# telin0411/multimodal_sequencing

Measured on AMD Instinct MI355X. Metric: multimodal steps/sec (fwd+bwd) at N=5 steps, seq=512, ViT-B/16; 1/2/4/8 GPU, higher is better.
Workload: dtype bf16; 1 GPU; config3: ViT-B/16 + 12x768 joint encoder + BERSON, N=5 steps, 20 pairs/story, pair seq 120+393=513; global_batch=32, stories_per_gpu=32, micro_batch=32, seq_len=513, parallelism=dp1

## Files before the change

multimodal_sequencing_amd/csrc/gemm256.hip:

```cpp
#include "gemm_common.h"

using namespace mmseq_gemm_detail;

namespace {

typedef unsigned short us;
__device__ __forceinline__ void ld8(const us* p, float* v) {
  const u16x8 u = *reinterpret_cast<const u16x8*>(p);
#pragma unroll
  for (int r = 0; r < 8; ++r) v[r] = bf2f(u[r]);
}
__device__ __forceinline__ void st8(us* p, const float* v) {
  u16x8 u;
#pragma unroll
  for (int r = 0; r < 8; ++r) u[r] = f2bf(v[r]);
  *reinterpret_cast<u16x8*>(p) = u;
}

struct EpiIn { u16x8 x; };
template <bool BWD, bool Q8 = false, bool CHK = true>
__device__ __forceinline__ EpiIn epi8_load(const GemmArgs& a, int m, int n) {
  EpiIn in;
  in.x = (u16x8){0, 0, 0, 0, 0, 0, 0, 0};
  if (CHK && (m >= a.M || n >= a.N)) return in;
  const int64_t off = (int64_t)m * (Q8 ? a.ldcb : a.ldc) + n;
  if (BWD) in.x = *reinterpret_cast<const u16x8*>(reinterpret_cast<const us*>(a.dact) + off);
  else if (a.resid) in.x = *reinterpret_cast<const u16x8*>(reinterpret_cast<const us*>(a.resid) + (int64_t)m * a.ldr + n);
  else if (a.accumulate) in.x = *reinterpret_cast<const u16x8*>(reinterpret_cast<const us*>(a.C) + off);
  return in;
}

struct EpiBias { f32x4 b0, b1; };
__device__ __forceinline__ EpiBias epi_bias(const GemmArgs& a, int n) {
  EpiBias b;
  b.b0 = b.b1 = (f32x4){0.f, 0.f, 0.f, 0.f};
  if (!a.bias || n >= a.N) return b;
  if ((((uintptr_t)a.bias) & 15) == 0) {
    b.b0 = *reinterpret_cast<const f32x4*>(a.bias + n);
    b.b1 = *reinterpret_cast<const f32x4*>(a.bias + n + 4);
  } else {
#pragma unroll
    for (int r = 0; r < 4; ++r) { b.b0[r] = a.bias[n + r]; b.b1[r] = a.bias[n + 4 + r]; }
  }
  asm volatile("" ::"v"(b.b0), "v"(b.b1));
  return b;
}

constexpr int DT_LO = 117 << 7;
constexpr int DT_N = 13 * 128;
__device__ __forceinline__ int dtab_index(unsigned short u) {
  const int a = min(max((int)(u & 0x7FFFu) - DT_LO, 0), DT_N - 1);
  return a + (int)(u >> 15) * DT_N;
}
template <int ACT>
__device__ __forceinline__ void dtab_fill(float MMSEQ_LDS* tab) {
  for (int e = threadIdx.x; e < 2 * DT_N; e += blockDim.x) {
    const unsigned short u = (unsigned short)(((e / DT_N) << 15) | (e % DT_N + DT_LO));
    tab[e] = act_bwd(ACT, bf2f(u));
  }
}

template <int ACT, bool BWD, bool XIN, bool DTAB = false, bool CHK = true>
__device__ __forceinline__ void epi8(const GemmArgs& a, int m, int n, f32x4 lo, f32x4 hi, const EpiIn& in,
                                     const EpiBias& bias, const float MMSEQ_LDS* dtab = nullptr) {
  if (CHK && (m >= a.M || n >= a.N)) return;
  float v[8];
  if (XIN) {
#pragma unroll
    for (int r = 0; r < 4; ++r) {
      v[r] = fmaf(lo[r], a.alpha, bias.b0[r]);
      v[4 + r] = fmaf(hi[r], a.alpha, bias.b1[r]);
    }
  } else {
    bias_alpha8(v, lo, hi, a.alpha, bias.b0, bias.b1);
  }
#ifdef MMSEQ_EPI_SINK
  const int64_t off = (int64_t)(m & 255) * a.ldc + n;
#else
  const int64_t off = (int64_t)m * a.ldc + n;
#endif
  if (BWD) {
    if (DTAB) {
#pragma unroll
      for (int r = 0; r < 8; ++r) v[r] *= dtab[dtab_index(in.x[r])];
    } else if (ACT == MMSEQ_ACT_GELU_ERF) {
#pragma unroll
      for (int r = 0; r < 8; ++r) v[r] *= gelu_sig_grad(bf2f(in.x[r]));
    } else {
#pragma unroll
      for (int r = 0; r < 8; ++r) v[r] *= act_bwd_fast(ACT, bf2f(in.x[r]));
    }
  } else if (ACT) {
    if (a.aux) st8(reinterpret_cast<us*>(a.aux) + off, v);
    if (ACT == MMSEQ_ACT_GELU_ERF) {
      gelu_sig8(v);
    } else {
#pragma unroll
      for (int r = 0; r < 8; ++r) v[r] = act_fwd_fast(ACT, v[r]);
    }
  }
  if (!BWD && a.drop.thr) {
    float dm[8];
    drop_mul_pairs<4>(a.drop, (uint64_t)m * a.N + n, dm);
#pragma unroll
    for (int r = 0; r < 8; ++r) v[r] *= dm[r];
  }
  if (XIN && !BWD) {
#pragma unroll
    for (int r = 0; r < 8; ++r) v[r] += bf2f(in.x[r]);
  }
  st8(reinterpret_cast<us*>(a.C) + off, v);
}

__device__ __forceinline__ void q8_scale_words(const GemmArgs& a, int mrow, int ncol,
                                               const uint8_t MMSEQ_LDS* sq, int lane) {
  const uint32_t w = *(const uint32_t MMSEQ_LDS*)(sq + 4 * lane);
  const int Mp = (a.M + 63) & ~63;
  if (mrow < Mp && ncol < a.N) {
    const int KB = a.N >> 5;
    const rsrc_t rq = make_rsrc(a.q8_scales, (int64_t)(Mp >> 6) * KB * 64);
    const uint32_t off = (uint32_t)(((mrow >> 6) * KB + (ncol >> 5)) * 64 + (mrow & 15) * 4);
    __builtin_amdgcn_raw_buffer_store_b32(w, rq, off, 0, 0);
  }
}
template <int ACT, bool BWD = false>
__device__ __forceinline__ void epi8_q8(const GemmArgs& a, int m, int n, int g, f32x4 lo, f32x4 hi,
                                        const EpiBias& bias, uint8_t MMSEQ_LDS* sqb,
                                        const EpiIn* din = nullptr,
                                        const float MMSEQ_LDS* dtab = nullptr) {
  float v[8];
  bias_alpha8(v, lo, hi, a.alpha, bias.b0, bias.b1);
  const bool in = m < a.M && n < a.N;
  const int64_t offb = (int64_t)m * a.ldcb + n;
  if (BWD) {
#pragma unroll
    for (int r = 0; r < 8; ++r) v[r] *= dtab[dtab_index(din->x[r])];
  } else {
    if (ACT && a.aux && in) st8(reinterpret_cast<us*>(a.aux) + offb, v);
    if (ACT == MMSEQ_ACT_GELU_ERF) {
      gelu_sig8(v);
    } else if (ACT) {
#pragma unroll
      for (int r = 0; r < 8; ++r) v[r] = act_fwd_fast(ACT, v[r]);
    }
  }
  float amax = 0.f;
#pragma unroll
  for (int r = 0; r < 8; ++r) {
    v[r] = bf2f(f2bf(v[r]));
    amax = fmaxf(amax, fabsf(v[r]));
  }
  if (a.cbf && in) st8(reinterpret_cast<us*>(a.cbf) + offb, v);
  {
    uint32_t u = __float_as_uint(amax);
    const auto r16 = __builtin_amdgcn_permlane16_swap(u, u, false, false);
    u = max(r16[0], r16[1]);
    const auto r32 = __builtin_amdgcn_permlane32_swap(u, u, false, false);
    amax = __uint_as_float(max(r32[0], r32[1]));
  }
  int e = amax > 0.f ? (int)((__float_as_uint(amax) >> 23) & 0xff) - 127 : -127;
  e = max(-127, min(127, e - 8));
  const float inv = ldexpf(1.f, -e);
  *sqb = (uint8_t)(m < a.M ? e + 127 : 0);
  if (!in) return;
  uint32_t w[2];
#pragma unroll
  for (int j = 0; j < 2; ++j) {
    const float s0 = fminf(448.f, fmaxf(-448.f, v[4 * j] * inv));
    const float s1 = fminf(448.f, fmaxf(-448.f, v[4 * j + 1] * inv));
    const float s2 = fminf(448.f, fmaxf(-448.f, v[4 * j + 2] * inv));
    const float s3 = fminf(448.f, fmaxf(-448.f, v[4 * j + 3] * inv));
    int pk = __builtin_amdgcn_cvt_pk_fp8_f32(s0, s1, 0, false);
    pk = __builtin_amdgcn_cvt_pk_fp8_f32(s2, s3, pk, true);
    w[j] = (uint32_t)pk;
  }
  typedef __attribute__((ext_vector_type(2))) unsigned int u32x2;
  *reinterpret_cast<u32x2*>(reinterpret_cast<uint8_t*>(a.C) + (int64_t)m * a.ldc + n) =
      (u32x2){w[0], w[1]};
}

constexpr int G_LDA_HALF = 16384;

#ifndef MMSEQ_NT_GROUP_M
#define MMSEQ_NT_GROUP_M 8
#endif
#ifndef MMSEQ_NT_GROUP_M_AUX
#define MMSEQ_NT_GROUP_M_AUX 16
#endif
__device__ __forceinline__ void tile_mn(int tile, int tiles_n, int ntiles, int& tm, int& tn,
                                        bool aux2 = false) {
  const int GM = tiles_n >= 8 ? (aux2 && tiles_n >= 12 ? MMSEQ_NT_GROUP_M_AUX : MMSEQ_NT_GROUP_M) : 1;
  if (GM <= 1) {
    tm = tile / tiles_n;
    tn = tile - tm * tiles_n;
    return;
  }
  const int tiles_m = ntiles / tiles_n;
  const int per = GM * tiles_n;
  const int grp = tile / per, first = grp * GM;
  const int gm = min(tiles_m - first, GM);
  const int r = tile - grp * per;
  tm = first + r % gm;
  tn = r / gm;
}

__device__ __forceinline__ int g8_of(int X, int q) {
  if (X == 0) return (q & 7) + ((q >> 3) << 4);
  if (X == 3) return 8 + (q & 7) + ((q >> 3) << 4);
  if (X == 1) return (q & 3) + ((q >> 2) << 3);
  return 4 + (q & 3) + ((q >> 2) << 3);
}

typedef __attribute__((ext_vector_type(8))) int i32x8;
typedef __attribute__((ext_vector_type(4))) int i32x4;
__device__ __forceinline__ i32x8 cat8(const bf16x8_t& lo, const bf16x8_t& hi) {
  const i32x4 l = __builtin_bit_cast(i32x4, lo), h = __builtin_bit_cast(i32x4, hi);
  return (i32x8){l[0], l[1], l[2], l[3], h[0], h[1], h[2], h[3]};
}

__device__ __forceinline__ void mfma_f8_acc(f32x4& c, const i32x8& a, const i32x8& b, uint32_t sa,
                                            uint32_t sb) {
  asm volatile("v_mfma_scale_f32_16x16x128_f8f6f4 %0, %1, %2, %0, %3, %4 op_sel_hi:[0,0,0]"
               : "+v"(c) : "v"(a), "v"(b), "v"(sa), "v"(sb));
}

template <int ACT, bool BWD, bool XIN, bool Q8 = false, bool F8 = false>
__global__ __launch_bounds__(512, 1) void gemm256_nt_kernel(GemmArgs a, int tiles_n, int ntiles,
                                                            int delay) {
  __shared__ __attribute__((aligned(16))) unsigned short
      smem[2 * 2 * G_LDA_HALF + (BWD ? 4 * DT_N : 0) + (F8 ? 2048 : 0) + 1024 + (Q8 ? 1024 : 0)];
  unsigned short* const sscale = smem + 2 * 2 * G_LDA_HALF + (BWD ? 4 * DT_N : 0);
  unsigned short* const sbias = smem + 2 * 2 * G_LDA_HALF + (BWD ? 4 * DT_N : 0) + (F8 ? 2048 : 0);
  const int tid = threadIdx.x, lane = tid & 63;
  const int wave = __builtin_amdgcn_readfirstlane(tid >> 6);
  uint8_t MMSEQ_LDS* const sq8 = (uint8_t MMSEQ_LDS*)(sbias + 1024) + wave * 256;
  const int wr = wave >> 2, wc = wave & 3;
  const int G = gridDim.x;
  const bool aux2 = ACT > 0 && !BWD && a.aux != nullptr;
  float MMSEQ_LDS* dtab = (float MMSEQ_LDS*)(smem + 2 * 2 * G_LDA_HALF);
  if (BWD) dtab_fill<ACT>(dtab);
  const int bid = blockIdx.x;
  const int first = xcd_item(bid, G);
  if (delay > 0 && first < ntiles && (ntiles - 1 - first) / G < (ntiles - 1) / G) {
    const uint64_t t0 = __builtin_amdgcn_s_memtime();
    while (__builtin_amdgcn_s_memtime() - t0 < (uint64_t)delay) __builtin_amdgcn_s_sleep(8);
  }
  const int nk = F8 ? a.K >> 7 : a.K >> 6;
  const int64_t lda_b = F8 ? a.lda : 2 * a.lda, ldb_b = F8 ? a.ldb : 2 * a.ldb;
  const int64_t kbytes = F8 ? a.K : 2 * a.K;
  const uint8_t* Ab = reinterpret_cast<const uint8_t*>(a.A);
  const uint8_t* Bb = reinterpret_cast<const uint8_t*>(a.B);
  const int KB32 = a.K >> 5;
  constexpr int LBUF = F8 ? G_LDA_HALF : 2 * G_LDA_HALF;
  constexpr int LOPB = F8 ? 2 * G_LDA_HALF : G_LDA_HALF;

  const int lr = lane >> 3, lc = lane & 7;
  const uint32_t offA0 = (uint32_t)(lr * lda_b + ((lc ^ (lane >> 4)) << 4));
  const uint32_t offA1 = (uint32_t)(lr * lda_b + ((lc ^ ((lane >> 4) | 4)) << 4));
  const uint32_t offB0 = (uint32_t)(lr * ldb_b + ((lc ^ ((lane >> 4) & 1)) << 4));
  const uint32_t offB1 = (uint32_t)(lr * ldb_b + ((lc ^ (((lane >> 4) & 1) | 2)) << 4));
  const uint32_t offB2 = (uint32_t)(lr * ldb_b + ((lc ^ (((lane >> 4) & 1) | 4)) << 4));
  const uint32_t offB3 = (uint32_t)(lr * ldb_b + ((lc ^ (((lane >> 4) & 1) | 6)) << 4));

  const rsrc_t rBias = make_rsrc(a.bias, a.bias ? (int64_t)a.N * 4 : 0);
  const rsrc_t rSA = make_rsrc(a.f8_sa, F8 ? a.f8_sa_bytes : 0);
  const rsrc_t rSB = make_rsrc(a.f8_sb, F8 ? a.f8_sb_bytes : 0);
  struct Sc { int ga, gb; };
  auto descs = [&](int tile, rsrc_t& ra, rsrc_t& rb, Sc& sc) {
    if (tile < ntiles) {
      int tm, tn;
      tile_mn(tile, tiles_n, ntiles, tm, tn, aux2);
      const int m0 = tm * 256, n0 = tn * 256;
      ra = make_rsrc(Ab + (int64_t)m0 * lda_b, (int64_t)(a.M - m0 - 1) * lda_b + kbytes);
      rb = make_rsrc(Bb + (int64_t)n0 * ldb_b, (int64_t)(a.N - n0 - 1) * ldb_b + kbytes);
      sc.ga = m0 >> 6;
      sc.gb = n0 >> 6;
    } else {
      ra = rb = make_rsrc(Ab, 0);
      sc.ga = (int)(a.f8_sa_bytes / 64 / (KB32 > 0 ? KB32 : 1));
      sc.gb = (int)(a.f8_sb_bytes / 64 / (KB32 > 0 ? KB32 : 1));
    }
  };
  rsrc_t rAc, rBc, rAn, rBn;
  Sc scc{}, scn{};
  descs(first, rAc, rBc, scc);
  descs(first + G, rAn, rBn, scn);

  auto stage = [&](int it, int kk, int X) {
    (void)it;
    const bool nxt = kk >= nk;
    if (nxt) kk -= nk;
    const bool isA = (X == 0 || X == 3);
    const rsrc_t r = isA ? (nxt ? rAn : rAc) : (nxt ? rBn : rBc);
    const int64_t ld = isA ? lda_b : ldb_b;
    unsigned short* img = smem + (kk & 1) * LBUF + (isA ? 0 : LOPB);
#pragma unroll
    for (int i = 0; i < 2; ++i) {
      const int q = wave * 2 + i;
      const int g8 = g8_of(X, q);
      const int gb = g8 & 3;
      const uint32_t lo = isA ? ((g8 & 1) ? offA1 : offA0)
                              : (gb == 0 ? offB0 : gb == 1 ? offB1 : gb == 2 ? offB2 : offB3);
      const uint32_t voff = lo + (uint32_t)(g8 * 8 * ld + kk * 128);
      dma16(r, img + g8 * 512, voff);
    }
    if (F8 && X == 3) {
      const bool sa = wave < 4;
      const int grp = (sa ? (nxt ? scn.ga : scc.ga) : (nxt ? scn.gb : scc.gb)) + (wave & 3);
      const uint32_t so = (uint32_t)(((int64_t)grp * KB32 + 4 * kk) * 64 + lane * 16);
      unsigned short* dst = sscale + (kk & 1) * 1024 + wave * 128;
      if (sa) {
        if (lane < 16) dma16(rSA, dst, so);
      } else {
        if (lane < 16) dma16(rSB, dst, so);
      }
    }
  };

  const int l15 = lane & 15;
  const int sw0 = ((lane >> 4) ^ (l15 >> 1)) << 3;
  const int sw1 = ((4 + (lane >> 4)) ^ (l15 >> 1)) << 3;
  const int arow = (wr * 128 + l15) * 64;
  const int hb = ((l15 >> 1) & 1) | ((l15 >> 2) << 1);
  const int swb0 = ((lane >> 4) ^ hb) << 3;
  const int swb1 = ((4 + (lane >> 4)) ^ hb) << 3;
  const int brow = LOPB + ((wc >> 1) * 128 + (wc & 1) * 64 + 8 * (l15 >> 2) + (l15 & 3)) * 64;
#define FR(base, t, ks) __builtin_bit_cast(bf16x8_t, *reinterpret_cast<const u16x8*>( \
      smem + (base) + (t) * 1024 + ((ks) ? sw1 : sw0)))
#define FRB(base, j, ks) __builtin_bit_cast(bf16x8_t, *reinterpret_cast<const u16x8*>( \
      smem + (base) + (4 * ((j) & 1) + 32 * ((j) >> 1)) * 64 + ((ks) ? swb1 : swb0)))

  uint32_t scA[2] = {0u, 0u}, scB[2] = {0u, 0u};
  const int scb_sh = 8 * (l15 >> 3);
  const uint8_t* scbase = reinterpret_cast<const uint8_t*>(sscale) + (lane >> 4) * 64;
  auto read_scales = [&](int h) {
    const uint8_t* sp = scbase + h * 2048;
    scA[0] = *reinterpret_cast<const uint32_t*>(sp + (wr * 2) * 256 + l15 * 4);
    scA[1] = *reinterpret_cast<const uint32_t*>(sp + (wr * 2 + 1) * 256 + l15 * 4);
    const int rb = 8 * ((l15 >> 2) & 1) + (l15 & 3);
    scB[0] = *reinterpret_cast<const uint32_t*>(sp + 1024 + wc * 256 + rb * 4);
    scB[1] = *reinterpret_cast<const uint32_t*>(sp + 1024 + wc * 256 + (rb + 4) * 4);
  };
#define QUAD(I0, I1, J0, J1)                                                                      \
  if (F8) {                                                                                       \
    uint32_t sa_[I1 - I0], sb_[J1 - J0];                                                          \
    _Pragma("unroll") for (int i = I0; i < I1; ++i) sa_[i - I0] = scA[i >> 2] >> (8 * (i & 3));   \
    _Pragma("unroll") for (int j = J0; j < J1; ++j)                                               \
      sb_[j - J0] = scB[j & 1] >> (scb_sh + 16 * (j >> 1));                                       \
        \
                                       \
    asm volatile("s_nop 4" ::"v"(sa_[0]), "v"(sa_[I1 - I0 - 1]), "v"(sb_[0]), "v"(sb_[J1 - J0 - 1])); \
    _Pragma("unroll") for (int i = I0; i < I1; ++i)                                               \
    _Pragma("unroll") for (int j = J0; j < J1; ++j)                                               \
      mfma_f8_acc(acc[i][j], fb8[j], fa8[i], sb_[j - J0], sa_[i - I0]);                           \
  } else {                                                                                        \
    _Pragma("unroll") for (int ks = 0; ks < 2; ++ks)                                              \
    _Pragma("unroll") for (int i = I0; i < I1; ++i)                                               \
    _Pragma("unroll") for (int j = J0; j < J1; ++j)                                               \
      acc[i][j] = __builtin_amdgcn_mfma_f32_16x16x32_bf16(fb[j][ks], fa[i][ks], acc[i][j], 0, 0, 0); \
  }

  int it = 0;
  if (first >= ntiles) return;
  stage(0, 0, 0); stage(0, 0, 1); stage(0, 0, 2); stage(0, 0, 3);
  stage(0, 1, 0); stage(0, 1, 1);
  asm volatile("s_waitcnt vmcnt(4)" ::: "memory");
  __builtin_amdgcn_s_barrier();
  if (wr) __builtin_amdgcn_s_barrier();

  f32x4 acc[8][4];
  bf16x8_t fa[8][2], fb[4][2];
  i32x8 fa8[8], fb8[4];
#define LDA(i)                                                                  \
  do {                                                                          \
    if (F8) fa8[i] = cat8(FR(buf + arow, i, 0), FR(buf + arow, i, 1));          \
    else { fa[i][0] = FR(buf + arow, i, 0); fa[i][1] = FR(buf + arow, i, 1); }  \
  } while (0)
#define LDB(j)                                                                  \
  do {                                                                          \
    if (F8) fb8[j] = cat8(FRB(buf + brow, j, 0), FRB(buf + brow, j, 1));        \
    else { fb[j][0] = FRB(buf + brow, j, 0); fb[j][1] = FRB(buf + brow, j, 1); } \
  } while (0)
  for (int tile = first; tile < ntiles; tile += G, ++it) {
#pragma unroll
    for (int i = 0; i < 8; ++i)
#pragma unroll
      for (int j = 0; j < 4; ++j) acc[i][j] = (f32x4){0.f, 0.f, 0.f, 0.f};
    if (ACT >= 0 && wave == 0) {
      uint32_t ln;
      asm volatile("v_mbcnt_lo_u32_b32 %0, -1, 0\n\tv_mbcnt_hi_u32_b32 %0, -1, %0" : "=v"(ln));
      dma16(rBias, sbias + (it & 1) * 512, (uint32_t)(scc.gb * 256) + ln * 16u);
    }

    for (int s = 0; s < (nk >> 1); ++s) {
#pragma unroll
      for (int h = 0; h < 2; ++h) {
        const int buf = h * LBUF;
#pragma unroll
        for (int i = 0; i < 4; ++i) LDA(i);
#pragma unroll
        for (int j = 0; j < 2; ++j) LDB(j);
        if (F8) read_scales(h);
        if (h == 0) stage(it, 2 * s + 1, 2); else stage(it, 2 * s + 2, 2);
        __builtin_amdgcn_sched_barrier(0);
        __builtin_amdgcn_s_barrier();
        asm volatile("s_waitcnt lgkmcnt(0)" ::: "memory");
        __builtin_amdgcn_sched_barrier(0);
        __builtin_amdgcn_s_setprio(1);
        QUAD(0, 4, 0, 2)
        __builtin_amdgcn_s_setprio(0);
        __builtin_amdgcn_sched_barrier(0);
        __builtin_amdgcn_s_barrier();
#pragma unroll
        for (int j = 2; j < 4; ++j) LDB(j);
        if (h == 0) stage(it, 2 * s + 1, 3); else stage(it, 2 * s + 2, 3);
        __builtin_amdgcn_sched_barrier(0);
        __builtin_amdgcn_s_barrier();
        asm volatile("s_waitcnt lgkmcnt(0)" ::: "memory");
        __builtin_amdgcn_sched_barrier(0);
        __builtin_amdgcn_s_setprio(1);
        QUAD(0, 4, 2, 4)
        __builtin_amdgcn_s_setprio(0);
        __builtin_amdgcn_sched_barrier(0);
        __builtin_amdgcn_s_barrier();
#pragma unroll
        for (int i = 4; i < 8; ++i) LDA(i);
        if (h == 0) stage(it, 2 * s + 2, 0); else stage(it, 2 * s + 3, 0);
        __builtin_amdgcn_sched_barrier(0);
        __builtin_amdgcn_s_barrier();
        asm volatile("s_waitcnt lgkmcnt(0)" ::: "memory");
        __builtin_amdgcn_sched_barrier(0);
        __builtin_amdgcn_s_setprio(1);
        QUAD(4, 8, 2, 4)
        __builtin_amdgcn_s_setprio(0);
        __builtin_amdgcn_sched_barrier(0);
        __builtin_amdgcn_s_barrier();
        if (h == 0) stage(it, 2 * s + 2, 1); else stage(it, 2 * s + 3, 1);
        __builtin_amdgcn_sched_barrier(0);
        asm volatile("s_waitcnt vmcnt(4)" ::: "memory");
        __builtin_amdgcn_s_barrier();
        __builtin_amdgcn_sched_barrier(0);
        __builtin_amdgcn_s_setprio(1);
        QUAD(4, 8, 0, 2)
        __builtin_amdgcn_s_setprio(0);
        __builtin_amdgcn_sched_barrier(0);
        __builtin_amdgcn_s_barrier();
      }
    }

    if (F8) asm volatile("s_nop 7\n\ts_nop 7\n\ts_nop 7\n\ts_nop 7" ::: "memory");
    int tm, tn;
    tile_mn(tile, tiles_n, ntiles, tm, tn, aux2);
    const int m0 = tm * 256, n0 = tn * 256;
    int lane_e = lane;
    if (Q8) asm volatile("v_mov_b32 %0, %1" : "=v"(lane_e) : "v"(lane));
    const int g = lane_e >> 4, ii = lane_e & 15;
    if (ACT < 0) {
#pragma unroll
      for (int i = 0; i < 8; ++i)
#pragma unroll
        for (int j = 0; j < 4; ++j) asm volatile("" ::"v"(acc[i][j]));
      rAc = rAn;
      rBc = rBn;
      scc = scn;
      descs(tile + 2 * G, rAn, rBn, scn);
      continue;
    }
    EpiBias bias0, bias1;
    {
      const float* sb = reinterpret_cast<const float*>(sbias + (it & 1) * 512) + wc * 64 + 8 * g;
      bias0.b0 = *reinterpret_cast<const f32x4*>(sb);
      bias0.b1 = *reinterpret_cast<const f32x4*>(sb + 4);
      bias1.b0 = *reinterpret_cast<const f32x4*>(sb + 32);
      bias1.b1 = *reinterpret_cast<const f32x4*>(sb + 36);
    }
    if (XIN) {
#define XIN_EPI(CHK_) \
      EpiIn in[2][2][2]; \
_Pragma("unroll") \
      for (int i = 0; i < 2; ++i) \
_Pragma("unroll") \
        for (int t = 0; t < 2; ++t) \
          in[0][i][t] = epi8_load<BWD, Q8, CHK_>(a, m0 + wr * 128 + i * 16 + ii, n0 + wc * 64 + 32 * t + 8 * g); \
_Pragma("unroll") \
      for (int h = 0; h < 4; ++h) { \
        if (h + 1 < 4) { \
_Pragma("unroll") \
          for (int i = 0; i < 2; ++i) \
_Pragma("unroll") \
            for (int t = 0; t < 2; ++t) \
              in[(h + 1) & 1][i][t] = epi8_load<BWD, Q8, CHK_>(a, m0 + wr * 128 + (2 * h + 2 + i) * 16 + ii, \
                                                     n0 + wc * 64 + 32 * t + 8 * g); \
        } \
        asm volatile("" ::"v"(in[h & 1][0][0].x), "v"(in[h & 1][0][1].x), "v"(in[h & 1][1][0].x), \
                     "v"(in[h & 1][1][1].x)); \
_Pragma("unroll") \
        for (int i = 0; i < 2; ++i) \
_Pragma("unroll") \
          for (int t = 0; t < 2; ++t) { \
            if (Q8 && BWD) \
              epi8_q8<ACT, true>(a, m0 + wr * 128 + (2 * h + i) * 16 + ii, n0 + wc * 64 + 32 * t + 8 * g, g, \
                                 acc[2 * h + i][2 * t], acc[2 * h + i][2 * t + 1], t ? bias1 : bias0, \
                                 sq8 + (((2 * h + i) >> 2) * 2 + t) * 64 + ii * 4 + ((2 * h + i) & 3), \
                                 &in[h & 1][i][t], dtab); \
            else \
              epi8<ACT, BWD, true, BWD, CHK_>(a, m0 + wr * 128 + (2 * h + i) * 16 + ii, n0 + wc * 64 + 32 * t + 8 * g, \
                                        acc[2 * h + i][2 * t], acc[2 * h + i][2 * t + 1], in[h & 1][i][t], \
                                        t ? bias1 : bias0, dtab); \
          } \
      }
#ifndef MMSEQ_EPI_CHECK_ALL
      if (!(Q8 && BWD) && (ACT == 0 || BWD) && m0 + 256 <= a.M && n0 + 256 <= a.N) {
        XIN_EPI(false)
      } else
#endif
      {
        XIN_EPI(true)
      }
#undef XIN_EPI
      if (Q8 && BWD)
        q8_scale_words(a, m0 + wr * 128 + (g >> 1) * 64 + ii, n0 + wc * 64 + 32 * (g & 1), sq8, lane_e);
    } else if (Q8) {
#pragma unroll
      for (int i = 0; i < 8; ++i)
#pragma unroll
        for (int t = 0; t < 2; ++t)
          epi8_q8<ACT>(a, m0 + wr * 128 + i * 16 + ii, n0 + wc * 64 + 32 * t + 8 * g, g,
                       acc[i][2 * t], acc[i][2 * t + 1], t ? bias1 : bias0,
                       sq8 + ((i >> 2) * 2 + t) * 64 + ii * 4 + (i & 3));
      q8_scale_words(a, m0 + wr * 128 + (g >> 1) * 64 + ii, n0 + wc * 64 + 32 * (g & 1), sq8, lane_e);
    } else {
      const EpiIn none = {(u16x8){0, 0, 0, 0, 0, 0, 0, 0}};
#ifndef MMSEQ_EPI_CHECK_ALL
      if (m0 + 256 <= a.M && n0 + 256 <= a.N) {
#pragma unroll
        for (int i = 0; i < 8; ++i)
#pragma unroll
          for (int t = 0; t < 2; ++t)
            epi8<ACT, BWD, false, false, false>(a, m0 + wr * 128 + i * 16 + ii, n0 + wc * 64 + 32 * t + 8 * g,
                                                acc[i][2 * t], acc[i][2 * t + 1], none, t ? bias1 : bias0);
      } else
#endif
#pragma unroll
      for (int i = 0; i < 8; ++i)
#pragma unroll
        for (int t = 0; t < 2; ++t)
          epi8<ACT, BWD, false>(a, m0 + wr * 128 + i * 16 + ii, n0 + wc * 64 + 32 * t + 8 * g,
                                acc[i][2 * t], acc[i][2 * t + 1], none, t ? bias1 : bias0);
    }
    rAc = rAn;
    rBc = rBn;
    scc = scn;
    descs(tile + 2 * G, rAn, rBn, scn);
  }
#undef FR
#undef FRB
#undef QUAD
#undef LDA
#undef LDB
  if (!wr) __builtin_amdgcn_s_barrier();
  asm volatile("s_waitcnt vmcnt(0)" ::: "memory");
}


__global__ __launch_bounds__(512, 1) void gemm256_tn_kernel(GemmArgs a, int tiles_n, int ntiles) {
  __shared__ __attribute__((aligned(16))) unsigned short smem[2 * 2 * G_LDA_HALF];
  const int tid = threadIdx.x, lane = tid & 63;
  const int wave = __builtin_amdgcn_readfirstlane(tid >> 6);
  const int wr = wave >> 2, wc = wave & 3;
  const int G = gridDim.x;
  const int bid = blockIdx.x;
  const int item = xcd_item(bid, G);
  const int split = item / ntiles, tile = item - split * ntiles;
  const int tm = tile / tiles_n, tn = tile - tm * tiles_n;
  const int m0 = tm * 256, n0 = tn * 256;
  const int kbeg = split * a.kchunk;
  const int kend = min(a.K, kbeg + a.kchunk);
  const int nk = (((kend - kbeg) + 127) >> 7) << 1;
  const unsigned short* Ab = reinterpret_cast<const unsigned short*>(a.A);
  const unsigned short* Bb = reinterpret_cast<const unsigned short*>(a.B);
  const rsrc_t ra = make_rsrc(Ab + (int64_t)kbeg * a.lda + m0,
                              ((int64_t)(kend - kbeg - 1) * a.lda + (a.M - m0)) * 2);
  const rsrc_t rb = make_rsrc(Bb + (int64_t)kbeg * a.ldb + n0,
                              ((int64_t)(kend - kbeg - 1) * a.ldb + (a.N - n0)) * 2);
  const rsrc_t rz = make_rsrc(Ab, 0);

  uint32_t offA[4], offB[4];
#pragma unroll
  for (int v = 0; v < 4; ++v) {
    const int rr = 2 * v + (lane >> 5);
    const int c = (lane & 31) ^ (rr << 1);
    offA[v] = (uint32_t)((lane >> 5) * a.lda * 2 + c * 16);
    offB[v] = (uint32_t)((lane >> 5) * a.ldb * 2 + c * 16);
  }
  auto stage = [&](int kk, int X) {
    const bool isA = (X & 1) == 0;
    const rsrc_t r = kk < nk ? (isA ? ra : rb) : rz;
    const int64_t ld = isA ? a.lda : a.ldb;
    unsigned short* img = smem + (kk & 1) * (2 * G_LDA_HALF) + (isA ? 0 : G_LDA_HALF);
#pragma unroll
    for (int i = 0; i < 2; ++i) {
      const int q = wave * 2 + i;
      const int row = (X >> 1) * 32 + 2 * q;
      const uint32_t lo = isA ? offA[q & 3] : offB[q & 3];
      const uint32_t voff = lo + (uint32_t)(((int64_t)kk * 64 + row) * ld * 2);
      dma16(r, img + row * 256, voff);
    }
  };

  const int g = lane >> 4, ii = lane & 15, qq = ii >> 2, pp = ii & 3;
  const int kr = 4 * g + qq, t8 = kr & 7;
  int fA[8], fB[4];
#pragma unroll
  for (int i = 0; i < 8; ++i)
    fA[i] = kr * 256 + (((wr * 16 + 2 * i + (pp >> 1)) ^ (t8 << 1)) << 3) + (pp & 1) * 4;
#pragma unroll
  for (int j = 0; j < 4; ++j)
    fB[j] = G_LDA_HALF + kr * 256 + (((wc * 8 + 2 * j + (pp >> 1)) ^ (t8 << 1)) << 3) + (pp & 1) * 4;
  auto frag = [&](int off) -> bf16x8_t {
    s16x4 lo = __builtin_amdgcn_ds_read_tr16_b64_v4i16((MMSEQ_LDS s16x4*)(smem + off));
    s16x4 hi = __builtin_amdgcn_ds_read_tr16_b64_v4i16((MMSEQ_LDS s16x4*)(smem + off + 16 * 256));
    typedef __attribute__((ext_vector_type(8))) short s16x8;
    s16x8 v = {lo[0], lo[1], lo[2], lo[3], hi[0], hi[1], hi[2], hi[3]};
    return __builtin_bit_cast(bf16x8_t, v);
  };

  f32x4 acc[8][4];
#pragma unroll
  for (int i = 0; i < 8; ++i)
#pragma unroll
    for (int j = 0; j < 4; ++j) acc[i][j] = (f32x4){0.f, 0.f, 0.f, 0.f};
  bf16x8_t fa[8], fb[4];
  const bool cs_split = a.cs_slab != nullptr;
  const bool do_cs = a.cs != nullptr && (cs_split || tn == 0);
  float cs0 = 0.f, cs1 = 0.f;
  auto cs_add = [&](float& dst, const bf16x8_t& f) {
    typedef __attribute__((ext_vector_type(4))) unsigned int u32x4;
    const u32x4 u = __builtin_bit_cast(u32x4, f);
    float t = 0.f;
#pragma unroll
    for (int e = 0; e < 4; ++e) t += __uint_as_float(u[e] << 16) + __uint_as_float(u[e] & 0xFFFF0000u);
    dst += t;
  };

  stage(0, 0); stage(0, 1); stage(0, 2); stage(0, 3);
  stage(1, 1); stage(1, 0);
  asm volatile("s_waitcnt vmcnt(4)" ::: "memory");
  __builtin_amdgcn_s_barrier();
  if (wr) __builtin_amdgcn_s_barrier();

#define TN_PHASE(READS, STAGE, VMWAIT, I0, KS)                                          \
  READS;                                                                                \
  STAGE;                                                                                \
  __builtin_amdgcn_sched_barrier(0);                                                    \
  if (VMWAIT) asm volatile("s_waitcnt vmcnt(4)" ::: "memory");                          \
  __builtin_amdgcn_s_barrier();                                                         \
  asm volatile("s_waitcnt lgkmcnt(0)" ::: "memory");                                    \
  if (do_cs && my_k) {   \
                           \
    if (wc == 0) cs_add((I0) ? cs1 : cs0, fa[(I0) + 0]);                                  \
    else if (wc == 1) cs_add((I0) ? cs1 : cs0, fa[(I0) + 1]);                             \
    else if (wc == 2) cs_add((I0) ? cs1 : cs0, fa[(I0) + 2]);                             \
    else cs_add((I0) ? cs1 : cs0, fa[(I0) + 3]);                                          \
  }                                                                                       \
  __builtin_amdgcn_sched_barrier(0);                                                    \
  __builtin_amdgcn_s_setprio(1);                                                        \
  _Pragma("unroll") for (int i = I0; i < I0 + 4; ++i)                                   \
  _Pragma("unroll") for (int j = 0; j < 4; ++j)                                         \
      acc[i][j] = __builtin_amdgcn_mfma_f32_16x16x32_bf16(fb[j], fa[i], acc[i][j], 0, 0, 0); \
  __builtin_amdgcn_s_setprio(0);                                                        \
  __builtin_amdgcn_sched_barrier(0);                                                    \
  __builtin_amdgcn_s_barrier();

  for (int s = 0; s < (nk >> 1); ++s) {
#pragma unroll
    for (int h = 0; h < 2; ++h) {
      const int buf = h * (2 * G_LDA_HALF);
      const bool my_k = !cs_split || (2 * s + h) % tiles_n == tn;
      TN_PHASE(
          { _Pragma("unroll") for (int i = 0; i < 4; ++i) fa[i] = frag(buf + fA[i]);
            _Pragma("unroll") for (int j = 0; j < 4; ++j) fb[j] = frag(buf + fB[j]); },
          { if (h == 0) stage(2 * s + 1, 3); else stage(2 * s + 2, 3); }, false, 0, 0)
      TN_PHASE({ _Pragma("unroll") for (int i = 4; i < 8; ++i) fa[i] = frag(buf + fA[i]); },
               { if (h == 0) stage(2 * s + 1, 2); else stage(2 * s + 2, 2); }, false, 4, 0)
      TN_PHASE(
          { _Pragma("unroll") for (int i = 0; i < 4; ++i) fa[i] = frag(buf + 32 * 256 + fA[i]);
            _Pragma("unroll") for (int j = 0; j < 4; ++j) fb[j] = frag(buf + 32 * 256 + fB[j]); },
          { if (h == 0) stage(2 * s + 2, 1); else stage(2 * s + 3, 1); }, false, 0, 1)
      TN_PHASE({ _Pragma("unroll") for (int i = 4; i < 8; ++i) fa[i] = frag(buf + 32 * 256 + fA[i]); },
               { if (h == 0) stage(2 * s + 2, 0); else stage(2 * s + 3, 0); }, true, 4, 1)
    }
  }
#undef TN_PHASE
  if (!wr) __builtin_amdgcn_s_barrier();
  asm volatile("s_waitcnt vmcnt(0)" ::: "memory");

  if (do_cs) {
    cs0 += __shfl_xor(cs0, 16, 64);
    cs0 += __shfl_xor(cs0, 32, 64);
    cs1 += __shfl_xor(cs1, 16, 64);
    cs1 += __shfl_xor(cs1, 32, 64);
    if (g == 0) {
#pragma unroll
      for (int q = 0; q < 2; ++q) {
        const int m = m0 + wr * 128 + (q * 4 + wc) * 16 + ii;
        const float v = q ? cs1 : cs0;
        if (m < a.M) {
          if (cs_split) a.cs_slab[((int64_t)split * tiles_n + tn) * a.M + m] = v;
          else a.cs[m] += v;
        }
      }
    }
  }
  float* C = a.splitk > 1 ? a.slab + (int64_t)split * a.M * a.N : reinterpret_cast<float*>(a.C);
  const int64_t ldc = a.splitk > 1 ? a.N : a.ldc;
  if (!(a.splitk == 1 && a.accumulate)) {
#pragma unroll
    for (int i = 0; i < 8; ++i)
#pragma unroll
      for (int j = 0; j < 4; ++j) {
        const int m = m0 + wr * 128 + i * 16 + ii;
        const int n = n0 + wc * 64 + j * 16 + 4 * g;
        if (m < a.M && n < a.N)
          *reinterpret_cast<f32x4*>(C + (int64_t)m * ldc + n) = acc[i][j];
      }
  } else {
    auto ld = [&](int i, int j) {
      const int m = m0 + wr * 128 + i * 16 + ii;
      const int n = n0 + wc * 64 + j * 16 + 4 * g;
      return (m < a.M && n < a.N) ? *reinterpret_cast<const f32x4*>(C + (int64_t)m * ldc + n)
                                  : (f32x4){0.f, 0.f, 0.f, 0.f};
    };
    f32x4 cin[2][4];
#pragma unroll
    for (int j = 0; j < 4; ++j) cin[0][j] = ld(0, j);
#pragma unroll
    for (int i = 0; i < 8; ++i) {
      if (i + 1 < 8) {
#pragma unroll
        for (int j = 0; j < 4; ++j) cin[(i + 1) & 1][j] = ld(i + 1, j);
      }
      asm volatile("" ::"v"(cin[i & 1][0]), "v"(cin[i & 1][1]), "v"(cin[i & 1][2]), "v"(cin[i & 1][3]));
#pragma unroll
      for (int j = 0; j < 4; ++j) {
        const int m = m0 + wr * 128 + i * 16 + ii;
        const int n = n0 + wc * 64 + j * 16 + 4 * g;
        if (m < a.M && n < a.N)
          *reinterpret_cast<f32x4*>(C + (int64_t)m * ldc + n) = acc[i][j] + cin[i & 1][j];
      }
    }
  }
}


constexpr int S2_STAGE = 256 * 32 + 128 * 32;

template <int ACT, bool BWD, bool XIN>
__global__ __launch_bounds__(256, 2) void gemm_nt_2b_kernel(GemmArgs a, int tiles_n, int ntiles,
                                                             int ) {
  __shared__ __attribute__((aligned(16))) unsigned short smem[3 * S2_STAGE];
  const int tid = threadIdx.x, lane = tid & 63;
  const int wave = __builtin_amdgcn_readfirstlane(tid >> 6);
  const int wr = wave >> 1, wc = wave & 1;
  const int G = gridDim.x;
  const int bid = blockIdx.x;
  const int first = xcd_item(bid, G);
  const int nk = a.K >> 5;
  const unsigned short* Ab = reinterpret_cast<const unsigned short*>(a.A);
  const unsigned short* Bb = reinterpret_cast<const unsigned short*>(a.B);

  const int sw = ((lane >> 5) & 1) << 1;
  const uint32_t offA = (uint32_t)((lane >> 2) * a.lda * 2 + (((lane & 3) ^ sw) << 4));
  const uint32_t offB = (uint32_t)((lane >> 2) * a.ldb * 2 + (((lane & 3) ^ sw) << 4));
  auto stage = [&](int it, int kk) {
    if (kk >= nk) { kk -= nk; ++it; }
    const int tile = first + it * G;
    rsrc_t ra, rb;
    if (tile < ntiles) {
      const int tm = tile / tiles_n, tn = tile - tm * tiles_n;
// ... 512 lines not shown
```

Baseline: 2.585 steps/s.

## Stage GEMM256 epilogue through per-wave LDS slots for full-line coalesced stores

```diff
diff --git a/multimodal_sequencing_amd/csrc/gemm256.hip b/multimodal_sequencing_amd/csrc/gemm256.hip
--- a/multimodal_sequencing_amd/csrc/gemm256.hip
+++ b/multimodal_sequencing_amd/csrc/gemm256.hip
@@ -60,56 +60,109 @@
   }
 }
 
+struct EpiOut { u16x8 c, aux; };
+__device__ __forceinline__ u16x8 pack8(const float* v) {
+  u16x8 u;
+#pragma unroll
+  for (int r = 0; r < 8; ++r) u[r] = f2bf(v[r]);
+  return u;
+}
+template <int ACT, bool BWD, bool XIN, bool DTAB = false>
+__device__ __forceinline__ EpiOut epi8_val(const GemmArgs& a, int m, int n, f32x4 lo, f32x4 hi, const EpiIn& in,
+                                           const EpiBias& bias, const float MMSEQ_LDS* dtab = nullptr) {
+  EpiOut o;
+  o.aux = (u16x8){0, 0, 0, 0, 0, 0, 0, 0};
+  float v[8];
+  if (XIN) {
+#pragma unroll
+    for (int r = 0; r < 4; ++r) {
+      v[r] = fmaf(lo[r], a.alpha, bias.b0[r]);
+      v[4 + r] = fmaf(hi[r], a.alpha, bias.b1[r]);
+    }
+  } else {
+    bias_alpha8(v, lo, hi, a.alpha, bias.b0, bias.b1);
+  }
+  if (BWD) {
+    if (DTAB) {
+#pragma unroll
+      for (int r = 0; r < 8; ++r) v[r] *= dtab[dtab_index(in.x[r])];
+    } else if (ACT == MMSEQ_ACT_GELU_ERF) {
+#pragma unroll
+      for (int r = 0; r < 8; ++r) v[r] *= gelu_sig_grad(bf2f(in.x[r]));
+    } else {
+#pragma unroll
+      for (int r = 0; r < 8; ++r) v[r] *= act_bwd_fast(ACT, bf2f(in.x[r]));
+    }
+  } else if (ACT) {
+    o.aux = pack8(v);
+    if (ACT == MMSEQ_ACT_GELU_ERF) {
+      gelu_sig8(v);
+    } else {
+#pragma unroll
+      for (int r = 0; r < 8; ++r) v[r] = act_fwd_fast(ACT, v[r]);
+    }
+  }
+  if (!BWD && a.drop.thr) {
+    float dm[8];
+    drop_mul_pairs<4>(a.drop, (uint64_t)m * a.N + n, dm);
+#pragma unroll
+    for (int r = 0; r < 8; ++r) v[r] *= dm[r];
+  }
+  if (XIN && !BWD) {
+#pragma unroll
+    for (int r = 0; r < 8; ++r) v[r] += bf2f(in.x[r]);
+  }
+  o.c = pack8(v);
+  return o;
+}
+
 template <int ACT, bool BWD, bool XIN, bool DTAB = false, bool CHK = true>
 __device__ __forceinline__ void epi8(const GemmArgs& a, int m, int n, f32x4 lo, f32x4 hi, const EpiIn& in,
                                      const EpiBias& bias, const float MMSEQ_LDS* dtab = nullptr) {
   if (CHK && (m >= a.M || n >= a.N)) return;
-  float v[8];
-  if (XIN) {
-#pragma unroll
-    for (int r = 0; r < 4; ++r) {
-      v[r] = fmaf(lo[r], a.alpha, bias.b0[r]);
-      v[4 + r] = fmaf(hi[r], a.alpha, bias.b1[r]);
-    }
-  } else {
-    bias_alpha8(v, lo, hi, a.alpha, bias.b0, bias.b1);
-  }
+  const EpiOut o = epi8_val<ACT, BWD, XIN, DTAB>(a, m, n, lo, hi, in, bias, dtab);
 #ifdef MMSEQ_EPI_SINK
   const int64_t off = (int64_t)(m & 255) * a.ldc + n;
 #else
   const int64_t off = (int64_t)m * a.ldc + n;
 #endif
-  if (BWD) {
-    if (DTAB) {
-#pragma unroll
-      for (int r = 0; r < 8; ++r) v[r] *= dtab[dtab_index(in.x[r])];
-    } else if (ACT == MMSEQ_ACT_GELU_ERF) {
-#pragma unroll
-      for (int r = 0; r < 8; ++r) v[r] *= gelu_sig_grad(bf2f(in.x[r]));
-    } else {
-#pragma unroll
-      for (int r = 0; r < 8; ++r) v[r] *= act_bwd_fast(ACT, bf2f(in.x[r]));
-    }
-  } else if (ACT) {
-    if (a.aux) st8(reinterpret_cast<us*>(a.aux) + off, v);
-    if (ACT == MMSEQ_ACT_GELU_ERF) {
-      gelu_sig8(v);
-    } else {
-#pragma unroll
-      for (int r = 0; r < 8; ++r) v[r] = act_fwd_fast(ACT, v[r]);
-    }
-  }
-  if (!BWD && a.drop.thr) {
-    float dm[8];
-    drop_mul_pairs<4>(a.drop, (uint64_t)m * a.N + n, dm);
-#pragma unroll
-    for (int r = 0; r < 8; ++r) v[r] *= dm[r];
-  }
-  if (XIN && !BWD) {
-#pragma unroll
-    for (int r = 0; r < 8; ++r) v[r] += bf2f(in.x[r]);
-  }
-  st8(reinterpret_cast<us*>(a.C) + off, v);
+  if (ACT && !BWD && a.aux) *reinterpret_cast<u16x8*>(reinterpret_cast<us*>(a.aux) + off) = o.aux;
+  *reinterpret_cast<u16x8*>(reinterpret_cast<us*>(a.C) + off) = o.c;
+}
+
+struct LineLane {
+  int w;
+  int r;
+};
+__device__ __forceinline__ LineLane line_lane(int lane) {
+  const int g = lane >> 4, ii = lane & 15, lr = lane >> 3, lc = lane & 7;
+  return {ii * 64 + ((g ^ (ii & 7)) << 3), lr * 64 + ((lc ^ lr) << 3)};
+}
+template <bool CHK>
+__device__ __forceinline__ void line_load(const GemmArgs& a, const us* src, int64_t ld, int md, int nd,
+                                          u16x8& x0, u16x8& x1) {
+  x0 = x1 = (u16x8){0, 0, 0, 0, 0, 0, 0, 0};
+  if (!CHK || (md < a.M && nd < a.N)) x0 = *reinterpret_cast<const u16x8*>(src);
+  if (!CHK || (md + 8 < a.M && nd < a.N)) x1 = *reinterpret_cast<const u16x8*>(src + 8 * ld);
+}
+__device__ __forceinline__ void line_get(us* slot, const LineLane& ll, u16x8 x0, u16x8 x1, EpiIn& i0,
+                                         EpiIn& i1) {
+  *reinterpret_cast<u16x8*>(slot + ll.r) = x0;
+  *reinterpret_cast<u16x8*>(slot + ll.r + 512) = x1;
+  i0.x = *reinterpret_cast<const u16x8*>(slot + ll.w);
+  i1.x = *reinterpret_cast<const u16x8*>(slot + (ll.w ^ 32));
+}
+struct LineOut { u16x8 q0, q1; us* dst; int md; };
+__device__ __forceinline__ void line_xchg(us* slot, const LineLane& ll, u16x8 p0, u16x8 p1, LineOut& o) {
+  *reinterpret_cast<u16x8*>(slot + ll.w) = p0;
+  *reinterpret_cast<u16x8*>(slot + (ll.w ^ 32)) = p1;
+  o.q0 = *reinterpret_cast<const u16x8*>(slot + ll.r);
+  o.q1 = *reinterpret_cast<const u16x8*>(slot + ll.r + 512);
+}
+template <bool CHK>
+__device__ __forceinline__ void line_store(const GemmArgs& a, const LineOut& o, int64_t ld, int nd) {
+  if (!CHK || (o.md < a.M && nd < a.N)) *reinterpret_cast<u16x8*>(o.dst) = o.q0;
+  if (!CHK || (o.md + 8 < a.M && nd < a.N)) *reinterpret_cast<u16x8*>(o.dst + 8 * ld) = o.q1;
 }
 
 __device__ __forceinline__ void q8_scale_words(const GemmArgs& a, int mrow, int ncol,
@@ -227,8 +280,9 @@
 template <int ACT, bool BWD, bool XIN, bool Q8 = false, bool F8 = false>
 __global__ __launch_bounds__(512, 1) void gemm256_nt_kernel(GemmArgs a, int tiles_n, int ntiles,
                                                             int delay) {
-  __shared__ __attribute__((aligned(16))) unsigned short
-      smem[2 * 2 * G_LDA_HALF + (BWD ? 4 * DT_N : 0) + (F8 ? 2048 : 0) + 1024 + (Q8 ? 1024 : 0)];
+  constexpr bool LINES = !Q8 && !F8 && ACT >= 0;
+  constexpr int SLOT_OFF = 2 * 2 * G_LDA_HALF + (BWD ? 4 * DT_N : 0) + (F8 ? 2048 : 0) + 1024 + (Q8 ? 1024 : 0);
+  __shared__ __attribute__((aligned(16))) unsigned short smem[SLOT_OFF + (LINES ? 8 * 1024 : 0)];
   unsigned short* const sscale = smem + 2 * 2 * G_LDA_HALF + (BWD ? 4 * DT_N : 0);
   unsigned short* const sbias = smem + 2 * 2 * G_LDA_HALF + (BWD ? 4 * DT_N : 0) + (F8 ? 2048 : 0);
   const int tid = threadIdx.x, lane = tid & 63;
@@ -453,7 +507,7 @@
     tile_mn(tile, tiles_n, ntiles, tm, tn, aux2);
     const int m0 = tm * 256, n0 = tn * 256;
     int lane_e = lane;
-    if (Q8) asm volatile("v_mov_b32 %0, %1" : "=v"(lane_e) : "v"(lane));
+    if (Q8 || LINES) asm volatile("v_mov_b32 %0, %1" : "=v"(lane_e) : "v"(lane));
     const int g = lane_e >> 4, ii = lane_e & 15;
     if (ACT < 0) {
 #pragma unroll
@@ -474,7 +528,83 @@
       bias1.b0 = *reinterpret_cast<const f32x4*>(sb + 32);
       bias1.b1 = *reinterpret_cast<const f32x4*>(sb + 36);
     }
-    if (XIN) {
+    if constexpr (LINES) {
+      us* const slot = smem + SLOT_OFF + wave * 1024;
+      const LineLane ll = line_lane(lane_e);
+      const int md0 = m0 + wr * 128 + (lane_e >> 3), nd = n0 + wc * 64 + 8 * (lane_e & 7);
+      us* const cd = reinterpret_cast<us*>(a.C) + (int64_t)md0 * a.ldc + nd;
+      us* const xd = reinterpret_cast<us*>(a.aux) + (int64_t)md0 * a.ldc + nd;
+      const bool interior = m0 + 256 <= a.M && n0 + 256 <= a.N;
+      constexpr bool PIPE = BWD || (ACT == 0 && !XIN);
+      LineOut pend;
+#define LINE_PUT(CHK_, HAVE_, DST_, MD_, P0_, P1_) \
+      { \
+        LineOut nxt; \
+        line_xchg(slot, ll, P0_, P1_, nxt); \
+        nxt.dst = DST_; \
+        nxt.md = MD_; \
+        if (!PIPE) line_store<CHK_>(a, nxt, a.ldc, nd); \
+        else if (HAVE_) line_store<CHK_>(a, pend, a.ldc, nd); \
+        if (PIPE) pend = nxt; \
+      }
+#define LINE_BLOCK(CHK_, I_, IN0_, IN1_) \
+      { \
+        const int mi = m0 + wr * 128 + (I_) * 16 + ii, ni = n0 + wc * 64 + 8 * g; \
+        const EpiOut o0 = epi8_val<ACT, BWD, XIN, BWD>(a, mi, ni, acc[I_][0], acc[I_][1], IN0_, bias0, dtab); \
+        const EpiOut o1 = epi8_val<ACT, BWD, XIN, BWD>(a, mi, ni + 32, acc[I_][2], acc[I_][3], IN1_, bias1, dtab); \
+        if (ACT && !BWD && a.aux) \
+          LINE_PUT(CHK_, (I_) > 0, xd + (int64_t)(I_) * 16 * a.ldc, md0 + (I_) * 16, o0.aux, o1.aux) \
+        LINE_PUT(CHK_, (I_) > 0 || (ACT && !BWD && a.aux), cd + (int64_t)(I_) * 16 * a.ldc, md0 + (I_) * 16, o0.c, o1.c) \
+      }
+      if constexpr (XIN) {
+        const int64_t ldx = !BWD && a.resid ? a.ldr : a.ldc;
+        const us* const xs = reinterpret_cast<const us*>(BWD ? a.dact : a.resid ? a.resid : a.C) +
+                             (int64_t)md0 * ldx + nd;
+#define XIN_LINES(CHK_, NB_) \
+        u16x8 raw[2][NB_][2]; \
+_Pragma("unroll") \
+        for (int i = 0; i < NB_; ++i) \
+          line_load<CHK_>(a, xs + (int64_t)i * 16 * ldx, ldx, md0 + i * 16, nd, raw[0][i][0], raw[0][i][1]); \
+_Pragma("unroll") \
+        for (int h = 0; h < 8 / NB_; ++h) { \
+          if (h + 1 < 8 / NB_) { \
+_Pragma("unroll") \
+            for (int i = 0; i < NB_; ++i) \
+              line_load<CHK_>(a, xs + (int64_t)(NB_ * (h + 1) + i) * 16 * ldx, ldx, \
+                              md0 + (NB_ * (h + 1) + i) * 16, nd, raw[(h + 1) & 1][i][0], raw[(h + 1) & 1][i][1]); \
+          } \
+_Pragma("unroll") \
+          for (int i = 0; i < NB_; ++i) asm volatile("" ::"v"(raw[h & 1][i][0]), "v"(raw[h & 1][i][1])); \
+_Pragma("unroll") \
+          for (int i = 0; i < NB_; ++i) { \
+            EpiIn in0, in1; \
+            line_get(slot, ll, raw[h & 1][i][0], raw[h & 1][i][1], in0, in1); \
+            LINE_BLOCK(CHK_, NB_ * h + i, in0, in1) \
+          } \
+        }
+        if ((ACT == 0 || BWD) && interior) {
+          XIN_LINES(false, 2)
+        } else {
+          XIN_LINES(true, 1)
+        }
+#undef XIN_LINES
+      } else {
+        const EpiIn none = {(u16x8){0, 0, 0, 0, 0, 0, 0, 0}};
+        if (interior) {
+#pragma unroll
+          for (int i = 0; i < 8; ++i) LINE_BLOCK(false, i, none, none)
+        } else {
+#pragma unroll
+          for (int i = 0; i < 8; ++i) LINE_BLOCK(true, i, none, none)
+        }
+      }
+#undef LINE_BLOCK
+#undef LINE_PUT
+      if constexpr (PIPE) {
+        if (interior) line_store<false>(a, pend, a.ldc, nd);
+        else line_store<true>(a, pend, a.ldc, nd);
+      }
+    } else if (XIN) {
 #define XIN_EPI(CHK_) \
       EpiIn in[2][2][2]; \
 _Pragma("unroll") \
```

After: 2.599 steps/s, median of 6. About the same (+0.6%).
